# tambetm/simple_dqn

Measured on NVIDIA H100. Metric: DQN training steps/sec (batch 32, 84x84x4), higher is better.
Workload: dtype f16x3-split (fp32 accumulate)

## Files before the change

### simple_dqn_b200/csrc/net_umma.cu

```cuda
#include "net.cuh"
#include "net_umma.cuh"
#include "umma.cuh"
#include "umma2.cuh"
#include "umma_mn.cuh"
#include "conv1_tma.cuh"

namespace b200 {

__device__ __forceinline__ void ld8(const float* p, float v[8]) {
  const float4 a = *reinterpret_cast<const float4*>(p);
  const float4 b = *reinterpret_cast<const float4*>(p + 4);
  v[0] = a.x; v[1] = a.y; v[2] = a.z; v[3] = a.w; v[4] = b.x; v[5] = b.y; v[6] = b.z; v[7] = b.w;
}
__device__ __forceinline__ void st8(float* p, const float v[8]) {
  *reinterpret_cast<float4*>(p) = make_float4(v[0], v[1], v[2], v[3]);
  *reinterpret_cast<float4*>(p + 4) = make_float4(v[4], v[5], v[6], v[7]);
}
__device__ __forceinline__ void zero8(float v[8]) {
#pragma unroll
  for (int i = 0; i < 8; ++i) v[i] = 0.f;
}

struct UmmaState {
  __half* h16[3][2] = {};
  int64_t h_elems[3] = {};
  __half* dz16[4] = {};
  int64_t dz_elems[4] = {};
  uint8_t* img_fwd[2][4] = {};
  int64_t img_fwd_bytes[4] = {};
  uint8_t* im2col1 = nullptr;
  uint8_t* img_dgr[3] = {};
};
static inline UmmaState* ust(b200dqn_net* n) { return static_cast<UmmaState*>(n->umma_state); }

struct PlanePair {
  __half* hi;
  int64_t lo_off;
};

__device__ __forceinline__ void store_f32_and_planes(float* f32, const PlanePair& pl, int64_t i, const float v[8]) {
  if (f32) st8(f32 + i, v);
  umma2::split8_planes(v, pl.hi + i, pl.hi + pl.lo_off + i);
}

struct V2Conv1Fwd {
  static constexpr int kBN = 32;
  static constexpr bool kAExact = true, kARowMajorThreads = true, kBRowMajorThreads = false;
  static constexpr int kAMode = umma2::kReg, kBMode = umma2::kBulk;
  static constexpr bool kStagedEpilogue = true, kDumpA = true, kPrefetch = false;
  uint8_t* im2col;
  const uint8_t* src[2];
  const int32_t* idx[2];
  int shift[2];
  const uint8_t* wimg[2];
  float* out[2];
  PlanePair out16[2];
  int rows;
  __device__ int M(int) const { return rows * kP1 * kP1; }
  __device__ int N(int) const { return kC1; }
  __device__ void krange(int, int& kb, int& ke) const { kb = 0; ke = kK1 / 64; }
  __device__ const uint8_t* a_row_ptr(int z, int m) const {
    if (m >= rows * kP1 * kP1) return nullptr;
    const int n = m / (kP1 * kP1), pq = m % (kP1 * kP1), p = pq / kP1, q = pq % kP1;
    const int64_t f = static_cast<int64_t>((z ? idx[1] : idx[0])[n]) + (z ? shift[1] : shift[0]);
    return (z ? src[1] : src[0]) + f * kFrameBytes + (p * 4) * kFrameW + q * 4;
  }
  __device__ uint2 a_raw8(const uint8_t* row, int k0) const {
    if (!row) return make_uint2(0u, 0u);
    const int c = k0 >> 6, r = (k0 >> 3) & 7;
    const uint8_t* ptr = row + c * kFrameBytes + r * kFrameW;
    return make_uint2(*reinterpret_cast<const uint32_t*>(ptr), *reinterpret_cast<const uint32_t*>(ptr + 4));
  }
  __device__ static void cvt8(uint2 raw, float v[8]) {
#pragma unroll
    for (int j = 0; j < 4; ++j) {
      v[j] = float((raw.x >> (8 * j)) & 0xffu);
      v[4 + j] = float((raw.y >> (8 * j)) & 0xffu);
    }
  }
  __device__ const uint8_t* b_tile(int z, int, int kb) const { return (z ? wimg[1] : wimg[0]) + kb * (kC1 * 256); }
  __device__ uint8_t* a_dump(int z, int mtile, int kb) const {
    return (z == 0 && im2col) ? im2col + (int64_t(mtile) * (kK1 / 64) + kb) * (128 * 128) : nullptr;
  }
  __device__ void store8(int z, int m, int n0, const float v[8]) const {
    float o[8];
#pragma unroll
    for (int j = 0; j < 8; ++j) o[j] = fmaxf(v[j] * (1.0f / 255.0f), 0.f);
    store_f32_and_planes(z ? out[1] : out[0], z ? out16[1] : out16[0], int64_t(m) * kC1 + n0, o);
  }
};

template <int H, int C, int R, int ST, int KO>
struct V2ConvFwd {
  static constexpr int P = (H - R) / ST + 1, K = R * R * C;
  static_assert(K % 64 == 0 && C % 8 == 0, "k-blocks of 64, chunks of 8 channels");
  static constexpr int kBN = KO;
  static constexpr bool kAExact = false, kARowMajorThreads = true, kBRowMajorThreads = false;
  static constexpr int kAMode = umma2::kAsync, kBMode = umma2::kBulk;
  static constexpr bool kStagedEpilogue = true, kDumpA = false, kPrefetch = false;
  PlanePair in16[2];
  const uint8_t* wimg[2];
  float* out[2];
  PlanePair out16[2];
  int rows;
  __device__ int M(int) const { return rows * P * P; }
  __device__ int N(int) const { return KO; }
  __device__ void krange(int, int& kb, int& ke) const { kb = 0; ke = K / 64; }
  __device__ umma2::Planes a_planes(int z) const { return {z ? in16[1].hi : in16[0].hi, in16[0].lo_off}; }
  __device__ umma2::RowCtx a_row(int, int m) const {
    const int n = m / (P * P), pq = m % (P * P), p = pq / P, q = pq % P;
    return {(int64_t(n * H + p * ST) * H + q * ST) * C, 0, 0, m < rows * P * P};
  }
  __device__ bool a_chunk(int, const umma2::RowCtx& rc, int kk, int64_t& off) const {
    const int r = kk / (R * C), sc = kk % (R * C);
    off = rc.base + r * (H * C) + sc;
    return true;
  }
  __device__ const uint8_t* b_tile(int z, int, int kb) const { return (z ? wimg[1] : wimg[0]) + kb * (KO * 256); }
  __device__ void store8(int z, int m, int n0, const float v[8]) const {
    float o[8];
#pragma unroll
    for (int j = 0; j < 8; ++j) o[j] = fmaxf(v[j], 0.f);
    store_f32_and_planes(z ? out[1] : out[0], z ? out16[1] : out16[0], int64_t(m) * KO + n0, o);
  }
};

struct V2Fc1Fwd {
  static constexpr int kBN = 32;
  static constexpr bool kAExact = false, kARowMajorThreads = false, kBRowMajorThreads = true;
  static constexpr int kAMode = umma2::kBulk, kBMode = umma2::kAsync;
  static constexpr bool kStagedEpilogue = false, kDumpA = false, kPrefetch = false;
  static constexpr bool kAMnMajor = true;
  static constexpr uint32_t kAMnLoOffset = 128 * 128;
  PlanePair in16[2];
  const uint8_t* wimg[2];
  float* part;
  int rows, splits;
  __device__ int M(int) const { return kHidden; }
  __device__ int N(int) const { return rows; }
  __device__ void krange(int z, int& kb, int& ke) const {
    const int per = (kFlat / 64 + splits - 1) / splits;
    kb = (z % splits) * per;
    ke = min(kb + per, kFlat / 64);
  }
  __device__ const uint8_t* a_sub(int z, int mtile, int kb, int chunk) const {
    return ((z / splits) ? wimg[1] : wimg[0]) + (int64_t(kb >> 1) * (kHidden / 64) + 2 * mtile + chunk) * (128 * 256) +
           (kb & 1) * (64 * 128);
  }
  __device__ umma2::Planes b_planes(int z) const { return {(z / splits) ? in16[1].hi : in16[0].hi, in16[0].lo_off}; }
  __device__ umma2::RowCtx b_row(int, int n) const { return {int64_t(n) * kFlat, 0, 0, n < rows}; }
  __device__ bool b_chunk(int, const umma2::RowCtx& rc, int kk, int64_t& off) const {
    off = rc.base + kk;
    return true;
  }
  __device__ void store8(int z, int m, int n0, const float v[8]) const {
#pragma unroll
    for (int j = 0; j < 8; ++j)
      if (n0 + j < rows) part[(z * rows + n0 + j) * kHidden + m] = v[j];
  }
};

struct V2Fc1Dgrad {
  static constexpr int kBN = 32;
  static constexpr bool kAExact = false, kARowMajorThreads = true, kBRowMajorThreads = true;
  static constexpr int kAMode = umma2::kBulk, kBMode = umma2::kAsync;
  static constexpr bool kStagedEpilogue = false, kDumpA = false, kPrefetch = true;
  const uint8_t* wimg;
  PlanePair dz4;
  const float* h3;
  float* dz3;
  PlanePair dz3_16;
  int rows;
  __device__ int M(int) const { return kFlat; }
  __device__ int N(int) const { return rows; }
  __device__ void krange(int, int& kb, int& ke) const { kb = 0; ke = kHidden / 64; }
  __device__ const uint8_t* a_tile(int, int mtile, int kb) const {
    return wimg + (int64_t(mtile) * (kHidden / 64) + kb) * (128 * 256);
  }
  __device__ umma2::Planes b_planes(int) const { return {dz4.hi, dz4.lo_off}; }
  __device__ umma2::RowCtx b_row(int, int n) const { return {int64_t(n) * kHidden, 0, 0, n < rows}; }
  __device__ bool b_chunk(int, const umma2::RowCtx& rc, int kk, int64_t& off) const {
    off = rc.base + kk;
    return true;
  }
  __device__ void prefetch8(int, int m, int n0, float pf[8]) const {
#pragma unroll
    for (int j = 0; j < 8; ++j) pf[j] = (n0 + j < rows) ? h3[int64_t(n0 + j) * kFlat + m] : 0.f;
  }
  __device__ void store8p(int, int m, int n0, const float v[8], const float pf[8]) const {
#pragma unroll
    for (int j = 0; j < 8; ++j)
      if (n0 + j < rows) {
        const int64_t i = int64_t(n0 + j) * kFlat + m;
        const float o = pf[j] > 0.f ? v[j] : 0.f;
        if (dz3) dz3[i] = o;
        __half h, l;
        umma2::split1(o, h, l);
        dz3_16.hi[i] = h;
        dz3_16.hi[dz3_16.lo_off + i] = l;
      }
  }
};

template <int H, int C, int R, int ST, int KO, int STG = 0>
struct V2ConvDgrad {
  static constexpr int kStagesOverride = STG;
  static constexpr int P = (H - R) / ST + 1, RT = R / ST, HC = (H + ST - 1) / ST, K = RT * RT * KO;
  static_assert(K % 64 == 0 && KO % 8 == 0, "k-blocks of 64");
  static constexpr int kBN = C;
  static constexpr bool kAExact = false, kARowMajorThreads = true, kBRowMajorThreads = true;
  static constexpr int kAMode = umma2::kAsync, kBMode = umma2::kBulk;
  static constexpr bool kStagedEpilogue = true, kDumpA = false, kPrefetch = true;
  PlanePair dz;
  const uint8_t* wimg;
  const float* x;
  float* dx;
  PlanePair dx16;
  int rows;
  __device__ int M(int) const { return rows * HC * HC; }
  __device__ int N(int) const { return C; }
  __device__ void krange(int, int& kb, int& ke) const { kb = 0; ke = K / 64; }
  __device__ umma2::Planes a_planes(int) const { return {dz.hi, dz.lo_off}; }
  __device__ umma2::RowCtx a_row(int z, int m) const {
    const int n = m / (HC * HC), yx = m % (HC * HC), yy = yx / HC, xx = yx % HC;
    const bool ok = m < rows * HC * HC && yy * ST + z / ST < H && xx * ST + z % ST < H;
    return {(int64_t(n * P + yy) * P + xx) * KO, yy, xx, ok};
  }
  __device__ bool a_chunk(int, const umma2::RowCtx& rc, int kk, int64_t& off) const {
    const int rp = kk / (RT * KO), sp = (kk / KO) % RT, ko = kk % KO;
    const int p = rc.y - rp, q = rc.x - sp;
    off = rc.base - (rp * P + sp) * KO + ko;
    return p >= 0 && p < P && q >= 0 && q < P;
  }
  __device__ const uint8_t* b_tile(int z, int, int kb) const { return wimg + (int64_t(z) * (K / 64) + kb) * (C * 256); }
  __device__ void prefetch8(int z, int m, int c0, float pf[8]) const {
    const int n = m / (HC * HC), yx = m % (HC * HC), yy = yx / HC, xx = yx % HC;
    const int y = yy * ST + z / ST, xq = xx * ST + z % ST;
    if (y >= H || xq >= H) { zero8(pf); return; }
    ld8(x + (int64_t(n * H + y) * H + xq) * C + c0, pf);
  }
  __device__ void store8p(int z, int m, int c0, const float v[8], const float xv[8]) const {
    const int n = m / (HC * HC), yx = m % (HC * HC), yy = yx / HC, xx = yx % HC;
    const int y = yy * ST + z / ST, xq = xx * ST + z % ST;
    if (y >= H || xq >= H) return;
    const int64_t i = (int64_t(n * H + y) * H + xq) * C + c0;
    float o[8];
#pragma unroll
    for (int j = 0; j < 8; ++j) o[j] = xv[j] > 0.f ? v[j] : 0.f;
    if (dx) st8(dx + i, o);
    if (dx16.hi) umma2::split8_planes(o, dx16.hi + i, dx16.hi + dx16.lo_off + i);
  }
};

template <int H, int C, int R, int ST, int KO>
struct WConvWgrad {
  static constexpr int P = (H - R) / ST + 1, KW = R * R * C;
  static_assert((R * C) % 64 == 0 && KO == 64, "64-element runs must not straddle a filter row");
  static constexpr int kBN = 64, kStages = 4;
  static constexpr bool kAExact = false, kABulk = false;
  PlanePair x16;
  PlanePair dz16;
  float* part;
  int rows, kb_per_split;
  __device__ int M(int) const { return KW; }
  __device__ int N(int) const { return KO; }
  __device__ void krange(int z, int& kb, int& ke) const {
    const int total = (rows * P * P + 63) / 64;
    kb = min(z * kb_per_split, total);
    ke = min(kb + kb_per_split, total);
  }
  __device__ umma_mn::PixCtx pix(int, int kpix) const {
    const int n = kpix / (P * P), pq = kpix % (P * P);
    return {n, pq / P, pq % P, kpix < rows * P * P};
  }
  __device__ umma2::Planes a_planes(int) const { return {x16.hi, x16.lo_off}; }
  __device__ bool a_run(int, const umma_mn::PixCtx& px, int mchunk, int64_t& off) const {
    const int m = mchunk * 64, r = m / (R * C), sc = m % (R * C);
    off = (int64_t(px.n * H + px.p * ST + r) * H + px.q * ST) * C + sc;
    return m < KW;
  }
  __device__ umma2::Planes b_planes(int) const { return {dz16.hi, dz16.lo_off}; }
  __device__ int64_t b_off(int, const umma_mn::PixCtx& px) const { return (int64_t(px.n * P + px.p) * P + px.q) * KO; }
  __device__ void store8(int z, int m, int n0, const float v[8]) const { st8(part + (int64_t(z) * KW + m) * KO + n0, v); }
};

struct WConv1Wgrad {
  static constexpr int kBN = 32, kStages = 4;
  static constexpr bool kAExact = true, kABulk = true;
  const uint8_t* im2col;
  PlanePair dz16;
  float* part;
  int rows, kb_per_split;
  int tile_rows;
  __device__ int M(int) const { return kK1; }
  __device__ int N(int) const { return kC1; }
  __device__ int total_kb() const {
    return tile_rows == 128 ? (rows * kP1 * kP1 + 63) / 64 : rows * conv1tma::kTilesPerSample * 2;
  }
  __device__ void krange(int z, int& kb, int& ke) const {
    const int total = total_kb();
    kb = min(z * kb_per_split, total);
    ke = min(kb + kb_per_split, total);
  }
  __device__ umma_mn::PixCtx pix(int, int kpix) const {
    if (tile_rows == 128) return {kpix, 0, 0, kpix < rows * kP1 * kP1};
    const int tile = kpix >> 7, local = kpix & 127;
    return {tile * tile_rows + local, 0, 0, local < tile_rows && tile < rows * conv1tma::kTilesPerSample};
  }
  __device__ const uint8_t* a_sub(int, int c, int kb) const {
    return im2col + (int64_t(kb >> 1) * (kK1 / 64) + c) * (128 * 128) + (kb & 1) * (64 * 128);
  }
  __device__ umma2::Planes b_planes(int) const { return {dz16.hi, dz16.lo_off}; }
  __device__ int64_t b_off(int, const umma_mn::PixCtx& px) const { return int64_t(px.n) * kC1; }
  __device__ void store8(int z, int m, int n0, const float v[8]) const {
    float o[8];
#pragma unroll
    for (int j = 0; j < 8; ++j) o[j] = v[j] * (1.0f / 255.0f);
    st8(part + (int64_t(z) * kK1 + m) * kC1 + n0, o);
  }
};

struct WFc1Wgrad {
  static constexpr int kBN = 64, kStages = 2;
  static constexpr bool kAExact = false, kABulk = false;
  PlanePair h3_16;
  PlanePair dz4_16;
  float* dw4;
  int rows;
  __device__ int M(int) const { return kFlat; }
  __device__ int N(int) const { return kHidden; }
  __device__ void krange(int, int& kb, int& ke) const { kb = 0; ke = (rows + 63) / 64; }
  __device__ umma_mn::PixCtx pix(int, int b) const { return {b, 0, 0, b < rows}; }
  __device__ umma2::Planes a_planes(int) const { return {h3_16.hi, h3_16.lo_off}; }
  __device__ bool a_run(int, const umma_mn::PixCtx& px, int mchunk, int64_t& off) const {
    off = int64_t(px.n) * kFlat + mchunk * 64;
    return mchunk * 64 < kFlat;
  }
  __device__ umma2::Planes b_planes(int) const { return {dz4_16.hi, dz4_16.lo_off}; }
  __device__ int64_t b_off(int, const umma_mn::PixCtx& px) const { return int64_t(px.n) * kHidden; }
  __device__ void store8(int, int m, int n0, const float v[8]) const { st8(dw4 + int64_t(m) * kHidden + n0, v); }
};

struct WFc1WgradGather {
  static constexpr int kBN = 64, kStages = 2;
  static constexpr bool kAExact = false, kABulk = false;
  const __half* h3g;
  const __half* dzg;
  int64_t h3_parity, h3_lo, dz_parity, dz_lo;
  const uint32_t* epoch;
  float* dw4;
  int rows;
  __device__ int M(int) const { return kFlat; }
  __device__ int N(int) const { return kHidden; }
  __device__ void krange(int, int& kb, int& ke) const { kb = 0; ke = (rows + 63) / 64; }
  __device__ umma_mn::PixCtx pix(int, int b) const { return {b, 0, 0, b < rows}; }
  __device__ umma2::Planes a_planes(int) const { return {h3g + int64_t(epoch[0] & 1) * h3_parity, h3_lo}; }
  __device__ bool a_run(int, const umma_mn::PixCtx& px, int mchunk, int64_t& off) const {
    off = int64_t(px.n) * kFlat + mchunk * 64;
    return mchunk * 64 < kFlat;
  }
  __device__ umma2::Planes b_planes(int) const { return {dzg + int64_t(epoch[1] & 1) * dz_parity, dz_lo}; }
  __device__ int64_t b_off(int, const umma_mn::PixCtx& px) const { return int64_t(px.n) * kHidden; }
  __device__ void store8(int, int m, int n0, const float v[8]) const { st8(dw4 + int64_t(m) * kHidden + n0, v); }
};

template <int K, int N>
struct PackFwdConv {
  static constexpr bool kRowMajorThreads = false;
  const float* w;
  __host__ __device__ int tiles() const { return 1; }
  __host__ __device__ int rows() const { return N; }
  __host__ __device__ int kblocks() const { return K / 64; }
  __device__ void src8(int, int r, int k0, float v[8]) const {
#pragma unroll
    for (int j = 0; j < 8; ++j) v[j] = w[(k0 + j) * N + r];
  }
};
struct PackFc1Dgrad {
  static constexpr bool kRowMajorThreads = true;
  const float* w;
  __host__ __device__ int tiles() const { return (kFlat + 127) / 128; }
  __host__ __device__ int rows() const { return 128; }
  __host__ __device__ int kblocks() const { return kHidden / 64; }
  __device__ void src8(int tile, int r, int k0, float v[8]) const {
    const int m = tile * 128 + r;
    if (m >= kFlat) { zero8(v); return; }
    ld8(w + m * kHidden + k0, v);
  }
};
template <int H, int C, int R, int ST, int KO>
struct PackConvDgrad {
  static constexpr int RT = R / ST, K = RT * RT * KO;
  static constexpr bool kRowMajorThreads = true;
  const float* w;
  __host__ __device__ int tiles() const { return ST * ST; }
  __host__ __device__ int rows() const { return C; }
  __host__ __device__ int kblocks() const { return K / 64; }
  __device__ void src8(int z, int c, int k0, float v[8]) const {
    const int rp = k0 / (RT * KO), sp = (k0 / KO) % RT, ko = k0 % KO;
    const int r = rp * ST + z / ST, s = sp * ST + z % ST;
    ld8(w + ((r * R + s) * C + c) * KO + ko, v);
  }
};

template <int KR, int N, bool DGRAD, int C, int R, int ST, bool XCHG = false>
__global__ void __launch_bounds__(256)
k_opt_conv(const float* __restrict__ part, int splits, float* __restrict__ w, float* __restrict__ sst,
           uint8_t* __restrict__ img_fwd, uint8_t* __restrict__ img_dgr, const OptArgs opt, const XllArgs x,
           const KTrace kt) {
  constexpr int64_t kSize = int64_t(KR) * N;
  kt_begin(kt);
  pdl_wait();
  pdl_launch_dependents();
  const int tid = threadIdx.x, lane8 = tid & 7;
  uint32_t epoch = 0;
  if constexpr (XCHG) epoch = *reinterpret_cast<volatile uint32_t*>(x.epoch + x.chan) + 1;
  const int64_t e4 = blockIdx.x * 32 + (tid >> 3);
  const int64_t i = e4 * 4;
  const bool live = i < kSize;
  float4 g = make_float4(0.f, 0.f, 0.f, 0.f);
  if (live) {
    const float* p = part + i;
    float4 v[8];
    int cnt = 0;
#pragma unroll
    for (int u = 0; u < 8; ++u) {
      const int sp = lane8 + 8 * u;
      if (sp < splits) { v[u] = *reinterpret_cast<const float4*>(p + sp * kSize); cnt = u + 1; }
    }
    for (int u = 0; u < cnt; ++u) { g.x += v[u].x; g.y += v[u].y; g.z += v[u].z; g.w += v[u].w; }
  }
#pragma unroll
  for (int o = 1; o < 8; o <<= 1) {
    g.x += __shfl_xor_sync(0xffffffffu, g.x, o);
    g.y += __shfl_xor_sync(0xffffffffu, g.y, o);
    g.z += __shfl_xor_sync(0xffffffffu, g.z, o);
    g.w += __shfl_xor_sync(0xffffffffu, g.w, o);
  }
  if constexpr (XCHG) {
    float4 v = lane8 == x.rank ? g : make_float4(0.f, 0.f, 0.f, 0.f);
    if (live && lane8 < x.world && lane8 != x.rank) {
      const int64_t par = int64_t(epoch & 1) * x.world * x.lines_per_src, el = (x.ll4 + e4) * 2;
      uint4* dst = x.recv[lane8] + par + int64_t(x.rank) * x.lines_per_src + el;
      st_ll(dst, __float_as_uint(g.x), __float_as_uint(g.y), epoch);
      st_ll(dst + 1, __float_as_uint(g.z), __float_as_uint(g.w), epoch);
      const uint4* src = x.recv[x.rank] + par + int64_t(lane8) * x.lines_per_src + el;
      ll_wait(src, epoch, x.err, v.x, v.y);
      ll_wait(src + 1, epoch, x.err, v.z, v.w);
    }
    __syncwarp();
    const int base = (tid & 31) & ~7;
    g = make_float4(0.f, 0.f, 0.f, 0.f);
    for (int p = 0; p < x.world; ++p) {
      const float a = __shfl_sync(0xffffffffu, v.x, base + p), b = __shfl_sync(0xffffffffu, v.y, base + p);
      const float c = __shfl_sync(0xffffffffu, v.z, base + p), d = __shfl_sync(0xffffffffu, v.w, base + p);
      if (p == 0) g = make_float4(a, b, c, d);
      else { g.x += a; g.y += b; g.z += c; g.w += d; }
    }
  }
  if (live && lane8 == 0) {
    float wp[4];
    opt_update_vec<4>(opt, opt_step_scalar(opt), reinterpret_cast<const float*>(&g), wp, w + i, sst + i);
    __half hi[4], lo[4];
#pragma unroll
    for (int j = 0; j < 4; ++j) umma2::split1(wp[j], hi[j], lo[j]);
    const int k = int(i / N), n0 = int(i % N);
    {
      uint8_t* base = img_fwd + int64_t(k / 64) * (N * 256) + (k % 8) * 2;
      const int c8 = (k % 64) / 8;
#pragma unroll
      for (int j = 0; j < 4; ++j) {
        const uint32_t off = umma::sw128_off(n0 + j, c8);
        *reinterpret_cast<__half*>(base + off) = hi[j];
        *reinterpret_cast<__half*>(base + N * 128 + off) = lo[j];
      }
    }
    if constexpr (DGRAD) {
      constexpr int RT = R / ST, NKB = RT * RT * N / 64;
      const int r = k / (R * C), s = (k / C) % R, c = k % C;
      const int z = (r % ST) * ST + (s % ST);
      const int kd = ((r / ST) * RT + (s / ST)) * N + n0;
      uint8_t* base = img_dgr + (int64_t(z) * NKB + kd / 64) * (C * 256) + umma::sw128_off(c, (kd % 64) / 8) + (kd % 8) * 2;
      *reinterpret_cast<uint2*>(base) = *reinterpret_cast<const uint2*>(hi);
      *reinterpret_cast<uint2*>(base + C * 128) = *reinterpret_cast<const uint2*>(lo);
    }
  }
  if constexpr (XCHG) {
    __syncthreads();
    if (tid == 0) {
      __threadfence();
      if (atomicAdd(x.ticket + x.chan, 1u) == gridDim.x - 1) {
        x.ticket[x.chan] = 0;
        __threadfence();
        *reinterpret_cast<volatile uint32_t*>(x.epoch + x.chan) = epoch;
      }
    }
  }
  kt_end(kt);
}

__global__ void __launch_bounds__(256)
k_opt_fc1(const float* __restrict__ dw, float* __restrict__ w, float* __restrict__ sst, uint8_t* __restrict__ img_dgr,
          const OptArgs opt, const KTrace kt) {
  kt_begin(kt);
  pdl_wait();
  pdl_launch_dependents();
  constexpr int kNB = kHidden / 8;
  const float l_step = opt_step_scalar(opt);
  for (int id = blockIdx.x * blockDim.x + threadIdx.x; id < kFlat * kNB; id += gridDim.x * blockDim.x) {
    const int m = id / kNB, n0 = (id % kNB) * 8;
    const int64_t i = int64_t(m) * kHidden + n0;
    float g[8], wv[8];
    ld8(dw + i, g);
    opt_update_vec<8>(opt, l_step, g, wv, w + i, sst + i);
    uint4 hi, lo;
    umma::split8(wv, hi, lo);
    uint8_t* base = img_dgr + (int64_t(m / 128) * (kHidden / 64) + n0 / 64) * (128 * 256) +
                    umma::sw128_off(m % 128, (n0 % 64) / 8);
    *reinterpret_cast<uint4*>(base) = hi;
    *reinterpret_cast<uint4*>(base + 128 * 128) = lo;
  }
  kt_end(kt);
}

int umma_opt_fc1(b200dqn_net* n, int rows, cudaStream_t st, bool from_g) {
  UmmaState* u = ust(n);
  const LayerTable& lt = n->lt;
  const float* dw = from_g ? n->d_g + lt.off[3] : n->d_part + lt.part_off[3];
  const int ctas = 2 * n->sm_count;
  B2_CHECK_CUDA(launch_pdl(k_opt_fc1, dim3(ctas), dim3(256), 0, st, dw, n->d_w + lt.off[3],
                           n->d_s + lt.off[3], u->img_dgr[0], make_opt_args(n, rows), ktrace_slot("opt_fc1")));
  B2_PROF("opt_fc1", st);
  return B200DQN_OK;
}

int umma_opt_conv(b200dqn_net* n, int l, int rows, cudaStream_t st, const char* label, bool from_g) {
  UmmaState* u = ust(n);
  const LayerTable& lt = n->lt;
  const OptArgs opt = make_opt_args(n, rows);
  const float* part = from_g ? n->d_g + lt.off[l] : n->d_part + lt.part_off[l];
  const int nsplits = from_g ? 1 : lt.splits[l];
  float* w = n->d_w + lt.off[l];
  float* s = n->d_s + lt.off[l];
  B2_REQUIRE(nsplits <= 64, B200DQN_EINVAL, "k_opt_conv handles at most 64 split-K partials");
  const int64_t size = lt.off[l + 1] - lt.off[l];
  const dim3 grid(unsigned((size / 4 + 31) / 32)), block(256);
  cudaError_t e;
  const XllArgs none{};
  if (l == 0)
    e = launch_pdl(k_opt_conv<kK1, kC1, false, 4, 8, 4>, grid, block, 0, st, part, nsplits, w, s, u->img_fwd[0][0],
                   (uint8_t*)nullptr, opt, none, ktrace_slot(label));
  else if (l == 1)
    e = launch_pdl(k_opt_conv<kK2, kC2, true, kC1, 4, 2>, grid, block, 0, st, part, nsplits, w, s, u->img_fwd[0][1],
                   u->img_dgr[2], opt, none, ktrace_slot(label));
  else
    e = launch_pdl(k_opt_conv<kK3, kC3, true, kC2, 3, 1>, grid, block, 0, st, part, nsplits, w, s, u->img_fwd[0][2],
                   u->img_dgr[1], opt, none, ktrace_slot(label));
  B2_CHECK_CUDA(e);
  B2_PROF(label, st);
  return B200DQN_OK;
}

int umma_opt_conv_xll(b200dqn_net* n, int l, int rows, cudaStream_t st, const char* label) {
  UmmaState* u = ust(n);
  const LayerTable& lt = n->lt;
  const OptArgs opt = make_opt_args(n, rows);
  B2_REQUIRE(l >= 0 && l < 3 && lt.splits[l] <= 64 && n->world <= 8, B200DQN_EINVAL, "opt_conv_xll: bad layer / world");
  XllArgs x{};
  int rc = comm_xll_args(n, l, &x);
  if (rc) return rc;
  const float* part = n->d_part + lt.part_off[l];
  float* w = n->d_w + lt.off[l];
  float* s = n->d_s + lt.off[l];
  const int64_t size = lt.off[l + 1] - lt.off[l];
  const dim3 grid(unsigned((size / 4 + 31) / 32)), block(256);
  cudaError_t e;
  if (l == 0)
    e = launch_pdl(k_opt_conv<kK1, kC1, false, 4, 8, 4, true>, grid, block, 0, st, part, lt.splits[l], w, s,
                   u->img_fwd[0][0], (uint8_t*)nullptr, opt, x, ktrace_slot(label));
  else if (l == 1)
    e = launch_pdl(k_opt_conv<kK2, kC2, true, kC1, 4, 2, true>, grid, block, 0, st, part, lt.splits[l], w, s,
                   u->img_fwd[0][1], u->img_dgr[2], opt, x, ktrace_slot(label));
  else
    e = launch_pdl(k_opt_conv<kK3, kC3, true, kC2, 3, 1, true>, grid, block, 0, st, part, lt.splits[l], w, s,
                   u->img_fwd[0][2], u->img_dgr[1], opt, x, ktrace_slot(label));
  B2_CHECK_CUDA(e);
  B2_PROF(label, st);
  return B200DQN_OK;
}

static int64_t fwd_image_bytes(int layer) {
  switch (layer) {
    case 0: return int64_t(kK1 / 64) * kC1 * 256;
    case 1: return int64_t(kK2 / 64) * kC2 * 256;
    case 2: return int64_t(kK3 / 64) * kC3 * 256;
    default: return int64_t((kFlat + 127) / 128) * (kHidden / 64) * 128 * 256;
  }
}

int umma_pack_layers(b200dqn_net* n, int which, int l0, int l1, cudaStream_t st) {
  if (n->cfg.math_mode != B200DQN_MATH_TCGEN05) return B200DQN_OK;
  UmmaState* u = ust(n);
  const LayerTable& lt = n->lt;
  const float* w = which ? n->d_tw : n->d_w;
  int rc = 0;
  for (int l = l0; l <= l1 && !rc; ++l) {
    switch (l) {
      case 0: rc = umma2::launch_pack("pack_c1", PackFwdConv<kK1, kC1>{w + lt.off[0]}, u->img_fwd[which][0], st); break;
      case 1:
        rc = umma2::launch_pack("pack_c2f", PackFwdConv<kK2, kC2>{w + lt.off[1]}, u->img_fwd[which][1], st);
        if (!rc && !which)
          rc = umma2::launch_pack("pack_c2d", PackConvDgrad<kP1, kC1, 4, 2, kC2>{w + lt.off[1]}, u->img_dgr[2], st);
        break;
      case 2:
        rc = umma2::launch_pack("pack_c3f", PackFwdConv<kK3, kC3>{w + lt.off[2]}, u->img_fwd[which][2], st);
        if (!rc && !which)
          rc = umma2::launch_pack("pack_c3d", PackConvDgrad<kP2, kC2, 3, 1, kC3>{w + lt.off[2]}, u->img_dgr[1], st);
        break;
      case 3:
        rc = umma2::launch_pack("pack_fc1", PackFc1Dgrad{w + lt.off[3]}, u->img_fwd[which][3], st);
        break;
      default: break;
    }
  }
  return rc;
}

static inline int fc1_splits_for(int rows) {
  static const int forced = getenv("B200DQN_FC1_SPLITS") ? atoi(getenv("B200DQN_FC1_SPLITS")) : 0;
  if (forced >= 1 && forced <= kFc1Splits) return forced;
  return rows <= 256 ? 7 : 4;
}
constexpr int kUWgradKb = 4;

static const bool g_conv1_tma = getenv("B200DQN_CONV1") && strcmp(getenv("B200DQN_CONV1"), "tma") == 0;
static inline int conv1_pixels_padded(int rows) { return g_conv1_tma ? rows * conv1tma::kTilesPerSample * 128 : rows * kP1 * kP1; }

int umma_wgrad_kb(int layer, int rows) {
  const int kred = layer == 0 ? conv1_pixels_padded(rows) : layer == 1 ? rows * kP2 * kP2 : rows * kP3 * kP3;
  const int kbs = (kred + 63) / 64;
  int per = (kbs + 47) / 48;
  if (layer == 0 && per < 8) per = 8;
  return per > kUWgradKb ? per : kUWgradKb;
}
int umma_wgrad_splits(int layer, int rows) {
  const int kred = layer == 0 ? conv1_pixels_padded(rows) : layer == 1 ? rows * kP2 * kP2 : rows * kP3 * kP3;
  const int kbs = (kred + 63) / 64, per = umma_wgrad_kb(layer, rows);
  return (kbs + per - 1) / per;
}

int umma_net_init(b200dqn_net* n) {
  if (n->cfg.math_mode != B200DQN_MATH_TCGEN05) return B200DQN_OK;
  auto* u = new UmmaState();
  n->umma_state = u;
  const int nb = n->nb;
  u->h_elems[0] = int64_t(nb) * kP1 * kP1 * kC1;
  u->h_elems[1] = int64_t(nb) * kP2 * kP2 * kC2;
  u->h_elems[2] = int64_t(nb) * kFlat;
  u->dz_elems[0] = int64_t(nb) * kHidden;
  u->dz_elems[1] = int64_t(nb) * kFlat;
  u->dz_elems[2] = int64_t(nb) * kP2 * kP2 * kC2;
  u->dz_elems[3] = int64_t(nb) * kP1 * kP1 * kC1;
  for (int i = 0; i < 3; ++i) {
    for (int z = 0; z < 2; ++z) {
      B2_CHECK_CUDA(cudaMalloc(&u->h16[i][z], 2 * u->h_elems[i] * sizeof(__half)));
      B2_CHECK_CUDA(cudaMemset(u->h16[i][z], 0, 2 * u->h_elems[i] * sizeof(__half)));
    }
  }
  for (int i = 0; i < 4; ++i) {
    B2_CHECK_CUDA(cudaMalloc(&u->dz16[i], 2 * u->dz_elems[i] * sizeof(__half)));
    B2_CHECK_CUDA(cudaMemset(u->dz16[i], 0, 2 * u->dz_elems[i] * sizeof(__half)));
  }
  for (int l = 0; l < 4; ++l) {
    u->img_fwd_bytes[l] = fwd_image_bytes(l);
    for (int z = 0; z < 2; ++z) {
      if (z == 1 && n->d_tw == n->d_w) { u->img_fwd[1][l] = u->img_fwd[0][l]; continue; }
      B2_CHECK_CUDA(cudaMalloc(&u->img_fwd[z][l], u->img_fwd_bytes[l]));
      B2_CHECK_CUDA(cudaMemset(u->img_fwd[z][l], 0, u->img_fwd_bytes[l]));
    }
  }
  B2_CHECK_CUDA(cudaMalloc(&u->im2col1, int64_t((conv1_pixels_padded(nb) + 127) / 128) * (kK1 / 64) * 128 * 128));
  u->img_dgr[0] = u->img_fwd[0][3];
  const int64_t dgr_bytes[3] = {0, int64_t(kK3 / 64) * kC2 * 256, int64_t(4) * (256 / 64) * kC1 * 256};
  for (int i = 1; i < 3; ++i) {
    B2_CHECK_CUDA(cudaMalloc(&u->img_dgr[i], dgr_bytes[i]));
    B2_CHECK_CUDA(cudaMemset(u->img_dgr[i], 0, dgr_bytes[i]));
  }
  return B200DQN_OK;
}

void umma_net_destroy(b200dqn_net* n) {
  UmmaState* u = ust(n);
  if (!u) return;
  for (int i = 0; i < 3; ++i) {
    for (int z = 0; z < 2; ++z) cudaFree(u->h16[i][z]);
    if (i > 0) cudaFree(u->img_dgr[i]);
  }
  for (int i = 0; i < 4; ++i) cudaFree(u->dz16[i]);
  cudaFree(u->im2col1);
  for (int l = 0; l < 4; ++l) {
    if (u->img_fwd[1][l] != u->img_fwd[0][l]) cudaFree(u->img_fwd[1][l]);
    cudaFree(u->img_fwd[0][l]);
  }
  delete u;
  n->umma_state = nullptr;
}

int umma_weights_changed(b200dqn_net* n, cudaStream_t st) {
  if (n->cfg.math_mode != B200DQN_MATH_TCGEN05) return B200DQN_OK;
  int rc = umma_pack_layers(n, 0, 0, 3, st);
  if (!rc && n->d_tw != n->d_w) rc = umma_pack_layers(n, 1, 0, 3, st);
  return rc;
}

int umma_target_synced(b200dqn_net* n, cudaStream_t st) {
  if (n->cfg.math_mode != B200DQN_MATH_TCGEN05 || n->d_tw == n->d_w) return B200DQN_OK;
  UmmaState* u = ust(n);
  for (int l = 0; l < 4; ++l)
    B2_CHECK_CUDA(cudaMemcpyAsync(u->img_fwd[1][l], u->img_fwd[0][l], u->img_fwd_bytes[l], cudaMemcpyDeviceToDevice, st));
  return B200DQN_OK;
}

void umma_dz4_planes(b200dqn_net* n, __half** hi, int64_t* lo_off) {
  UmmaState* u = ust(n);
  *hi = u ? u->dz16[0] : nullptr;
  *lo_off = u ? u->dz_elems[0] : 0;
}

int umma_forward(b200dqn_net* n, const uint8_t* const src[2], const int32_t* const idx[2], const int shift[2],
                 const int64_t nframes[2], int nets, int rows, cudaStream_t st, bool release_early) {
  UmmaState* u = ust(n);
  int rc;
  auto planes = [&](int i, int z) { return PlanePair{u->h16[i][z], u->h_elems[i]}; };
  if (g_conv1_tma) {
    conv1tma::Params p{};
    const bool shared5 = nets == 2 && src[0] == src[1] && idx[0] == idx[1] && shift[1] == shift[0] + 1;
    for (int z = 0; z < 2; ++z) {
      p.idx[z] = idx[z]; p.shift[z] = shift[z];
      p.wimg[z] = u->img_fwd[z][0]; p.out16[z] = u->h16[0][z];
    }
    p.out[0] = n->d_h1[0];
    p.out[1] = nullptr;
    p.shared5 = shared5 ? 1 : 0; p.nets = nets; p.rows = rows; p.lo_off = u->h_elems[0];
    p.im2col = (nets == 2 && rows == n->nb) ? u->im2col1 : nullptr;
    CUtensorMap m0, m1;
    const int64_t nframes0 = nframes[0], nframes1 = nframes[1];
    if ((rc = conv1tma::make_frame_map(&m0, src[0], nframes0, shared5 ? kHist + 1 : kHist))) return rc;
    if ((rc = conv1tma::make_frame_map(&m1, src[nets == 2 ? 1 : 0], nets == 2 ? nframes1 : nframes0, kHist))) return rc;
    static bool configured = false;
    if (!configured) {
      B2_CHECK_CUDA(cudaFuncSetAttribute(conv1tma::k_conv1_tma, cudaFuncAttributeMaxDynamicSharedMemorySize,
                                         int(conv1tma::smem_bytes(2))));
      configured = true;
    }
    const uint32_t smem = conv1tma::smem_bytes((nets == 2 && !shared5) ? 2 : 1);
    B2_CHECK_CUDA(launch_pdl(conv1tma::k_conv1_tma, dim3(rows * conv1tma::kTilesPerSample), dim3(umma2::kThreads2),
                             smem, st, m0, m1, p, ktrace_slot("conv1_fwd")));
    B2_PROF("conv1_fwd", st);
  } else {
    V2Conv1Fwd p;
    for (int z = 0; z < 2; ++z) {
      p.src[z] = src[z]; p.idx[z] = idx[z]; p.shift[z] = shift[z];
      p.wimg[z] = u->img_fwd[z][0]; p.out[z] = n->d_h1[z]; p.out16[z] = planes(0, z);
    }
    p.rows = rows;
    p.im2col = (nets == 2 && rows == n->nb) ? u->im2col1 : nullptr;
    if ((rc = umma2::launch_umma2("conv1_fwd", p, rows * kP1 * kP1, kC1, nets, st, release_early))) return rc;
  }
  {
    using P = V2ConvFwd<kP1, kC1, 4, 2, kC2>;
    P p;
    for (int z = 0; z < 2; ++z) {
      p.in16[z] = planes(0, z); p.wimg[z] = u->img_fwd[z][1]; p.out16[z] = planes(1, z);
      p.out[z] = z ? nullptr : n->d_h2[z];
    }
    p.rows = rows;
    if ((rc = umma2::launch_umma2("conv2_fwd", p, rows * kP2 * kP2, kC2, nets, st, false))) return rc;
  }
  {
    using P = V2ConvFwd<kP2, kC2, 3, 1, kC3>;
    P p;
    for (int z = 0; z < 2; ++z) {
      p.in16[z] = planes(1, z); p.wimg[z] = u->img_fwd[z][2]; p.out16[z] = planes(2, z);
      p.out[z] = z ? nullptr : n->d_h3[z];
    }
    p.rows = rows;
    if ((rc = umma2::launch_umma2("conv3_fwd", p, rows * kP3 * kP3, kC3, nets, st, release_early))) return rc;
    if (nets == 2 && rows == n->nb && comm_gather_active(n, st) && (rc = umma_push_h3(n, st))) return rc;
  }
  {
    V2Fc1Fwd p;
    for (int z = 0; z < 2; ++z) { p.in16[z] = planes(2, z); p.wimg[z] = u->img_fwd[z][3]; }
    p.part = n->d_fc1part; p.rows = rows; p.splits = fc1_splits_for(rows);
    if ((rc = umma2::launch_umma2("fc1_fwd", p, kHidden, rows, nets * p.splits, st, false))) return rc;
  }
  return B200DQN_OK;
}

int umma_backward_op(b200dqn_net* n, int op, const uint8_t* src, const int32_t* idx, int shift, int rows,
                     cudaStream_t st, bool release_early) {
  const LayerTable& lt = n->lt;
  const float* w = n->d_w;
  switch (op) {
    case 0: {
      UmmaState* u = ust(n);
      WFc1Wgrad p{PlanePair{u->h16[2][0], u->h_elems[2]}, PlanePair{u->dz16[0], u->dz_elems[0]},
                  n->d_part + lt.part_off[3], rows};
      return umma_mn::launch_umma_mn("fc1_wgrad", p, kFlat, kHidden, 1, st, release_early);
    }
    case 1: {
      UmmaState* u = ust(n);
      V2Fc1Dgrad p{u->img_dgr[0], PlanePair{u->dz16[0], u->dz_elems[0]}, n->d_h3[0], n->keep_grads ? n->d_dz3 : nullptr,
                   PlanePair{u->dz16[1], u->dz_elems[1]}, rows};
      return umma2::launch_umma2("fc1_dgrad", p, kFlat, rows, 1, st, release_early);
    }
    case 2: {
      UmmaState* u = ust(n);
      using P = WConvWgrad<kP2, kC2, 3, 1, kC3>;
      P p{PlanePair{u->h16[1][0], u->h_elems[1]}, PlanePair{u->dz16[1], u->dz_elems[1]},
          n->d_part + lt.part_off[2], rows, umma_wgrad_kb(2, rows)};
      return umma_mn::launch_umma_mn("conv3_wgrad", p, P::KW, kC3, lt.splits[2], st, release_early);
    }
    case 3: {
      UmmaState* u = ust(n);
      using P = V2ConvDgrad<kP2, kC2, 3, 1, kC3>;
      P p{PlanePair{u->dz16[1], u->dz_elems[1]}, u->img_dgr[1], n->d_h2[0], n->keep_grads ? n->d_dz2 : nullptr,
          PlanePair{u->dz16[2], u->dz_elems[2]}, rows};
      return umma2::launch_umma2("conv3_dgrad", p, rows * P::HC * P::HC, kC2, 1, st, release_early);
    }
    case 4: {
      UmmaState* u = ust(n);
      using P = WConvWgrad<kP1, kC1, 4, 2, kC2>;
      P p{PlanePair{u->h16[0][0], u->h_elems[0]}, PlanePair{u->dz16[2], u->dz_elems[2]},
          n->d_part + lt.part_off[1], rows, umma_wgrad_kb(1, rows)};
      return umma_mn::launch_umma_mn("conv2_wgrad", p, P::KW, kC2, lt.splits[1], st, release_early);
    }
    case 5: {
      UmmaState* u = ust(n);
      using P = V2ConvDgrad<kP1, kC1, 4, 2, kC2>;
      using P2 = V2ConvDgrad<kP1, kC1, 4, 2, kC2, 2>;
      if (n->world == 1) {
        P2 p{PlanePair{u->dz16[2], u->dz_elems[2]}, u->img_dgr[2], n->d_h1[0], n->keep_grads ? n->d_dz1 : nullptr,
             PlanePair{u->dz16[3], u->dz_elems[3]}, rows};
        return umma2::launch_umma2("conv2_dgrad", p, rows * P::HC * P::HC, kC1, 4, st, release_early);
      }
      P p{PlanePair{u->dz16[2], u->dz_elems[2]}, u->img_dgr[2], n->d_h1[0], n->keep_grads ? n->d_dz1 : nullptr,
          PlanePair{u->dz16[3], u->dz_elems[3]}, rows};
      return umma2::launch_umma2("conv2_dgrad", p, rows * P::HC * P::HC, kC1, 4, st, release_early);
    }
    default: {
      UmmaState* u = ust(n);
      (void)src; (void)idx; (void)shift;
      WConv1Wgrad p{u->im2col1, PlanePair{u->dz16[3], u->dz_elems[3]}, n->d_part + lt.part_off[0], rows,
                    umma_wgrad_kb(0, rows), g_conv1_tma ? conv1tma::kTileRows : 128};
      return umma_mn::launch_umma_mn("conv1_wgrad", p, kK1, kC1, lt.splits[0], st, release_early);
    }
  }
}

int umma_fc1_splits(int rows) { return fc1_splits_for(rows); }
int umma_push_h3(b200dqn_net* n, cudaStream_t st) {
  UmmaState* u = ust(n);
  cudaStream_t sN = n->side[3];
  B2_CHECK_CUDA(cudaEventRecord(n->ev[13], st));
  B2_CHECK_CUDA(cudaStreamWaitEvent(sN, n->ev[13], 0));
  const int rc = comm_push_planes(n, 0, u->h16[2][0], u->h_elems[2], sN);
  if (rc) return rc;
  B2_CHECK_CUDA(cudaEventRecord(n->ev[14], sN));
  return B200DQN_OK;
}
int umma_push_dz4(b200dqn_net* n, cudaStream_t st) {
  UmmaState* u = ust(n);
  return comm_push_planes(n, 1, u->dz16[0], u->dz_elems[0], st);
}
int umma_gather_dz4_ll(b200dqn_net* n, cudaStream_t st) {
  UmmaState* u = ust(n);
  return comm_gather_dz4_ll(n, u->dz16[0], u->dz_elems[0], st, true);
}
int umma_fc1_wgrad_gathered(b200dqn_net* n, cudaStream_t st) {
  WFc1WgradGather p{reinterpret_cast<const __half*>(n->d_xbuf + n->x_h3_off),
                    reinterpret_cast<const __half*>(n->d_xbuf + n->x_dz_off),
                    n->x_h3_parity / 2, n->x_h3_lo, n->x_dz_parity / 2, n->x_dz_lo,
                    n->d_xpush_epoch, n->d_part + n->lt.part_off[3], n->nb * n->world};
  return umma_mn::launch_umma_mn("fc1_wgrad", p, kFlat, kHidden, 1, st, false);
}

}

extern "C" int b200dqn_debug_trace(unsigned long long* host_out, int n) {
  cudaDeviceSynchronize();
  return b200::umma2::read_trace(host_out, n);
}
```

Before: 10740.

## Fuse conv2 and conv3 forward into one per-sample kernel keeping h2 in shared memory

Adds a fused conv23 forward kernel that runs one block per sample and net. It computes conv2 with a pipelined wgmma ring, keeps the ReLU'd h2 hi/lo planes in shared memory, and streams the conv3 weights into the retired ring stages before running conv3 from shared memory. The aim is to remove one kernel launch and the global round trip of h2 for batches of up to 64 rows. In exchange each block uses a large amount of shared memory, the grid is only rows x nets blocks, and the h2 planes are written to global only for net 0.

```diff
diff --git a/simple_dqn_b200/csrc/net_umma.cu b/simple_dqn_b200/csrc/net_umma.cu
--- a/simple_dqn_b200/csrc/net_umma.cu
+++ b/simple_dqn_b200/csrc/net_umma.cu
@@ -124,6 +124,260 @@
     store_f32_and_planes(z ? out[1] : out[0], z ? out16[1] : out16[0], int64_t(m) * KO + n0, o);
   }
 };
+
+struct Conv23Fwd {
+  using C2 = V2ConvFwd<kP1, kC1, 4, 2, kC2>;
+  using C3 = V2ConvFwd<kP2, kC2, 3, 1, kC3>;
+  C2 c2;
+  C3 c3;
+};
+
+namespace conv23 {
+constexpr int kStages = 4;
+constexpr int kM2 = kP2 * kP2, kM3 = kP3 * kP3;
+constexpr int kKb2 = kK2 / 64, kKb3 = kK3 / 64;
+constexpr uint32_t kA2 = umma::kBM * 128;
+constexpr uint32_t kB2 = kC2 * 128;
+constexpr uint32_t kStage2 = 2 * kA2 + 2 * kB2;
+constexpr uint32_t kB3 = kC3 * 256;
+constexpr uint32_t kA3 = umma::kWgM * 128;
+constexpr uint32_t kStaging = 3 * kStage2;
+constexpr uint32_t kH2 = kStages * kStage2;
+constexpr uint32_t kPitch2 = kC2 * 4 + 16, kPitch3 = kC3 * 4 + 16;
+constexpr uint32_t kSmemBytes = kH2 + 2 * kM2 * 128 + 1024;
+static_assert(kKb3 * kB3 == 3 * kStage2, "stages 0-2 of the conv2 ring hold the nine conv3 weight images");
+static_assert(kStaging + umma::kBM * kPitch2 <= kH2 && kStaging + 3 * 2 * kA3 <= kH2, "stage 3: epilogue tile, A ring");
+static_assert(umma::kWgM * kPitch3 <= kStaging, "conv3 epilogue tile over the retired weight images");
+static_assert(kSmemBytes <= 227 * 1024, "H100: at most 227 KB of shared memory per block");
+}
+
+__global__ void __launch_bounds__(umma2::kThreads2, 1) k_conv23_fwd(const Conv23Fwd p, const int trace_in,
+                                                                    const KTrace kt) {
+  using namespace conv23;
+  using umma2::g_trace;
+  using umma2::kTraceSlots;
+  constexpr int S = kStages;
+  constexpr int kThreads = umma2::kThreads2;
+  extern __shared__ uint8_t smem_raw[];
+  __shared__ __align__(8) uint64_t s_full[S];
+  __shared__ __align__(8) uint64_t s_w3[kKb3];
+
+  const int tid = threadIdx.x, warp = tid >> 5, lane = tid & 31, wg = warp >> 2;
+  const int n = blockIdx.x, z = blockIdx.y;
+  const bool trace = trace_in && n == 0 && z == 0;
+  kt_begin(kt);
+  B2_TRACE(tid == 0, 0);
+  const uint32_t smem_base = (smem_u32(smem_raw) + 1023u) & ~1023u;
+  uint8_t* smem_gen = smem_raw + (smem_base - smem_u32(smem_raw));
+  uint8_t* h2 = smem_gen + kH2;
+  const uint8_t* wimg2 = z ? p.c2.wimg[1] : p.c2.wimg[0];
+  const uint8_t* wimg3 = z ? p.c3.wimg[1] : p.c3.wimg[0];
+
+  if (tid == 0) {
+#pragma unroll
+    for (int s = 0; s < S; ++s) mbar_init(&s_full[s], kThreads + 1);
+#pragma unroll
+    for (int kb = 0; kb < kKb3; ++kb) mbar_init(&s_w3[kb], 1);
+    mbar_fence_init();
+  }
+  __syncthreads();
+  B2_TRACE(tid == 0, 1);
+
+  constexpr int kACh = umma::kBM * 8 / kThreads;
+  umma2::RowCtx arow[kACh];
+  const umma2::Planes apl = p.c2.a_planes(z);
+#pragma unroll
+  for (int i = 0; i < kACh; ++i) {
+    const int m = (tid + i * kThreads) >> 3;
+    arow[i] = p.c2.a_row(z, n * kM2 + m);
+    arow[i].ok = m < kM2;
+  }
+  if (tid == 0) {
+#pragma unroll
+    for (int j = 0; j < S; ++j) {
+      mbar_arrive_expect_tx(&s_full[j], 2 * kB2);
+      tma_bulk_g2s(smem_gen + j * kStage2 + 2 * kA2, wimg2 + j * (2 * kB2), 2 * kB2, &s_full[j]);
+    }
+  }
+  pdl_wait();
+
+  auto stage2 = [&](int j) {
+    const int s = j % S, k0 = j * umma::kBK;
+    B2_TRACE(tid == 0, 8 + j * 4 + 2);
+    const uint32_t a_hi = smem_base + s * kStage2, a_lo = a_hi + kA2;
+    if (tid == 0 && j >= S) {
+      mbar_arrive_expect_tx(&s_full[s], 2 * kB2);
+      tma_bulk_g2s(smem_gen + s * kStage2 + 2 * kA2, wimg2 + j * (2 * kB2), 2 * kB2, &s_full[s]);
+    }
+#pragma unroll
+    for (int i = 0; i < kACh; ++i) {
+      const int id = tid + i * kThreads, r = id >> 3, c = id & 7;
+      int64_t eoff = 0;
+      const bool ok = arow[i].ok && p.c2.a_chunk(z, arow[i], k0 + c * 8, eoff);
+      const uint32_t bytes = ok ? 16u : 0u;
+      const __half* hi = apl.hi + (ok ? eoff : 0);
+      const uint32_t off = umma::sw128_off(r, c);
+      umma2::cp_async16(a_hi + off, hi, bytes);
+      umma2::cp_async16(a_lo + off, hi + apl.lo_off, bytes);
+    }
+    umma2::cp_async_arrive_noinc(&s_full[s]);
+    B2_TRACE(tid == 0, 8 + j * 4 + 3);
+  };
+  for (int j = 0; j < S; ++j) stage2(j);
+
+  float acc[kC2];
+  float acc2[kC2 / 2];
+#pragma unroll
+  for (int i = 0; i < kC2; ++i) acc[i] = 0.f;
+#pragma unroll
+  for (int i = 0; i < kC2 / 2; ++i) acc2[i] = 0.f;
+  for (int it = 0; it < kKb2; ++it) {
+    const int s = it % S;
+    mbar_wait(&s_full[s], (it / S) & 1);
+    fence_proxy_async_smem();
+    B2_TRACE(tid == 0, 8 + it * 4 + 0);
+    const uint32_t sa = smem_base + s * kStage2;
+    const uint64_t da_hi = umma::make_desc_sw128(sa + wg * umma::kWgM * 128);
+    const uint64_t da_lo = umma::make_desc_sw128(sa + kA2 + wg * umma::kWgM * 128);
+    const uint64_t db = umma::make_desc_sw128(sa + 2 * kA2);
+    umma::wgmma_fence();
+#pragma unroll
+    for (int k = 0; k < umma::kBK / 16; ++k) {
+      umma::wgmma_f16<2 * kC2>(acc, da_hi + 2 * k, db + 2 * k);
+      umma::wgmma_f16<kC2>(acc2, da_lo + 2 * k, db + 2 * k);
+    }
+    umma::wgmma_commit();
+    umma::wgmma_wait<1>();
+    B2_TRACE(tid == 0, 8 + it * 4 + 1);
+    if (it >= 1) {
+      umma2::named_bar_sync(1, kThreads);
+      const int freed = (it - 1) % S;
+      if (it - 1 + S < kKb2) {
+        stage2(it - 1 + S);
+      } else if (tid == 0) {
+#pragma unroll
+        for (int t = 0; t < 3; ++t) {
+          const int kb = 3 * freed + t;
+          mbar_arrive_expect_tx(&s_w3[kb], kB3);
+          tma_bulk_g2s(smem_gen + kb * kB3, wimg3 + kb * kB3, kB3, &s_w3[kb]);
+        }
+      }
+    }
+  }
+  B2_TRACE(tid == 0, 3);
+  pdl_launch_dependents();
+
+  umma::wgmma_wait<0>();
+  umma2::named_bar_sync(1, kThreads);
+  B2_TRACE(tid == 0, 4);
+  umma::stage_acc<kC2>(acc, acc2, smem_gen + kStaging, kPitch2, wg, warp, lane);
+  umma2::named_bar_sync(1, kThreads);
+  {
+    float* out = p.c2.out[0];
+    const PlanePair pl = p.c2.out16[0];
+#pragma unroll
+    for (int i = 0; i < umma::kBM * 8 / kThreads; ++i) {
+      const int id = tid + i * kThreads, r = id >> 3, cc = id & 7;
+      if (r < kM2) {
+        const uint8_t* src = smem_gen + kStaging + r * kPitch2 + cc * 32;
+        const float4 v0 = *reinterpret_cast<const float4*>(src), v1 = *reinterpret_cast<const float4*>(src + 16);
+        const float v[8] = {v0.x, v0.y, v0.z, v0.w, v1.x, v1.y, v1.z, v1.w};
+        float o[8];
+#pragma unroll
+        for (int j = 0; j < 8; ++j) o[j] = fmaxf(v[j], 0.f);
+        uint4 hi, lo;
+        umma::split8(o, hi, lo);
+        *reinterpret_cast<uint4*>(h2 + r * 128 + cc * 16) = hi;
+        *reinterpret_cast<uint4*>(h2 + kM2 * 128 + r * 128 + cc * 16) = lo;
+        if (z == 0) {
+          const int64_t e = int64_t(n * kM2 + r) * kC2 + cc * 8;
+          if (out) st8(out + e, o);
+          *reinterpret_cast<uint4*>(pl.hi + e) = hi;
+          *reinterpret_cast<uint4*>(pl.hi + pl.lo_off + e) = lo;
+        }
+      }
+    }
+  }
+  umma2::named_bar_sync(1, kThreads);
+  B2_TRACE(tid == 0, 2);
+
+  float acc3[kC3 / 2];
+  float acc3l[kC3 / 4];
+#pragma unroll
+  for (int i = 0; i < kC3 / 2; ++i) acc3[i] = 0.f;
+#pragma unroll
+  for (int i = 0; i < kC3 / 4; ++i) acc3l[i] = 0.f;
+  for (int it = 0; it < kKb3; ++it) {
+    const int r = it / 3, s = it % 3;
+    const uint32_t a_off = kStaging + (it % 3) * (2 * kA3);
+    B2_TRACE(tid == 0, 8 + (kKb2 + it) * 4 + 2);
+#pragma unroll
+    for (int i = 0; i < umma::kWgM * 8 / kThreads; ++i) {
+      const int id = tid + i * kThreads, m = id >> 3, c = id & 7;
+      uint4 hi = make_uint4(0u, 0u, 0u, 0u), lo = hi;
+      if (m < kM3) {
+        const int src = (m / kP3 + r) * kP2 + m % kP3 + s;
+        hi = *reinterpret_cast<const uint4*>(h2 + src * 128 + c * 16);
+        lo = *reinterpret_cast<const uint4*>(h2 + kM2 * 128 + src * 128 + c * 16);
+      }
+      *reinterpret_cast<uint4*>(smem_gen + a_off + umma::sw128_off(m, c)) = hi;
+      *reinterpret_cast<uint4*>(smem_gen + a_off + kA3 + umma::sw128_off(m, c)) = lo;
+    }
+    fence_proxy_async_smem();
+    umma2::named_bar_sync(1, kThreads);
+    mbar_wait(&s_w3[it], 0);
+    B2_TRACE(tid == 0, 8 + (kKb2 + it) * 4 + 0);
+    const uint64_t da_hi = umma::make_desc_sw128(smem_base + a_off);
+    const uint64_t da_lo = umma::make_desc_sw128(smem_base + a_off + kA3);
+    const uint32_t b = smem_base + it * kB3 + wg * 32 * 128;
+    const uint64_t db_hi = umma::make_desc_sw128(b), db_lo = umma::make_desc_sw128(b + kC3 * 128);
+    umma::wgmma_fence();
+#pragma unroll
+    for (int k = 0; k < umma::kBK / 16; ++k) {
+      umma::wgmma_f16<32>(acc3, da_hi + 2 * k, db_hi + 2 * k);
+      umma::wgmma_f16<32>(acc3 + kC3 / 4, da_hi + 2 * k, db_lo + 2 * k);
+      umma::wgmma_f16<32>(acc3l, da_lo + 2 * k, db_hi + 2 * k);
+    }
+    umma::wgmma_commit();
+    umma::wgmma_wait<1>();
+    B2_TRACE(tid == 0, 8 + (kKb2 + it) * 4 + 1);
+  }
+
+  umma::wgmma_wait<0>();
+  umma2::named_bar_sync(1, kThreads);
+  B2_TRACE(tid == 0, 7);
+  umma::stage_acc<32>(acc3, acc3l, smem_gen + wg * 32 * 4, kPitch3, 0, warp, lane);
+  umma2::named_bar_sync(1, kThreads);
+#pragma unroll
+  for (int i = 0; i < umma::kWgM * 8 / kThreads; ++i) {
+    const int id = tid + i * kThreads, m = id >> 3, cc = id & 7;
+    if (m < kM3) {
+      const uint8_t* src = smem_gen + m * kPitch3 + cc * 32;
+      const float4 v0 = *reinterpret_cast<const float4*>(src), v1 = *reinterpret_cast<const float4*>(src + 16);
+      const float v[8] = {v0.x, v0.y, v0.z, v0.w, v1.x, v1.y, v1.z, v1.w};
+      p.c3.store8(z, n * kM3 + m, cc * 8, v);
+    }
+  }
+  B2_TRACE(tid == 0, 5);
+  kt_end(kt);
+  B2_TRACE(tid == 0, 6);
+}
+
+constexpr int kConv23MaxRows = 64;
+
+static int launch_conv23(const Conv23Fwd& p, int rows, int nets, cudaStream_t st) {
+  static bool configured = false;
+  if (!configured) {
+    B2_CHECK_CUDA(cudaFuncSetAttribute(k_conv23_fwd, cudaFuncAttributeMaxDynamicSharedMemorySize, conv23::kSmemBytes));
+    configured = true;
+  }
+  static const char* trace_label = getenv("B200DQN_TRACE_LABEL");
+  const int trace = (trace_label && strcmp(trace_label, "conv23_fwd") == 0) ? 1 : 0;
+  B2_CHECK_CUDA(launch_pdl(k_conv23_fwd, dim3(rows, nets), dim3(umma2::kThreads2), conv23::kSmemBytes, st, p, trace,
+                           ktrace_slot("conv23_fwd")));
+  B2_PROF("conv23_fwd", st);
+  return B200DQN_OK;
+}
 
 struct V2Fc1Fwd {
   static constexpr int kBN = 32;
@@ -767,27 +1021,39 @@
     p.im2col = (nets == 2 && rows == n->nb) ? u->im2col1 : nullptr;
     if ((rc = umma2::launch_umma2("conv1_fwd", p, rows * kP1 * kP1, kC1, nets, st, release_early))) return rc;
   }
-  {
-    using P = V2ConvFwd<kP1, kC1, 4, 2, kC2>;
-    P p;
+  if (rows <= kConv23MaxRows) {
+    Conv23Fwd p{};
     for (int z = 0; z < 2; ++z) {
-      p.in16[z] = planes(0, z); p.wimg[z] = u->img_fwd[z][1]; p.out16[z] = planes(1, z);
-      p.out[z] = z ? nullptr : n->d_h2[z];
-    }
-    p.rows = rows;
-    if ((rc = umma2::launch_umma2("conv2_fwd", p, rows * kP2 * kP2, kC2, nets, st, false))) return rc;
-  }
-  {
-    using P = V2ConvFwd<kP2, kC2, 3, 1, kC3>;
-    P p;
-    for (int z = 0; z < 2; ++z) {
-      p.in16[z] = planes(1, z); p.wimg[z] = u->img_fwd[z][2]; p.out16[z] = planes(2, z);
-      p.out[z] = z ? nullptr : n->d_h3[z];
-    }
-    p.rows = rows;
-    if ((rc = umma2::launch_umma2("conv3_fwd", p, rows * kP3 * kP3, kC3, nets, st, release_early))) return rc;
-    if (nets == 2 && rows == n->nb && comm_gather_active(n, st) && (rc = umma_push_h3(n, st))) return rc;
-  }
+      p.c2.in16[z] = planes(0, z); p.c2.wimg[z] = u->img_fwd[z][1];
+      p.c3.wimg[z] = u->img_fwd[z][2]; p.c3.out16[z] = planes(2, z);
+      p.c3.out[z] = z ? nullptr : n->d_h3[z];
+    }
+    p.c2.out[0] = n->d_h2[0]; p.c2.out16[0] = planes(1, 0);
+    p.c2.rows = p.c3.rows = rows;
+    if ((rc = launch_conv23(p, rows, nets, st))) return rc;
+  } else {
+    {
+      using P = V2ConvFwd<kP1, kC1, 4, 2, kC2>;
+      P p;
+      for (int z = 0; z < 2; ++z) {
+        p.in16[z] = planes(0, z); p.wimg[z] = u->img_fwd[z][1]; p.out16[z] = planes(1, z);
+        p.out[z] = z ? nullptr : n->d_h2[z];
+      }
+      p.rows = rows;
+      if ((rc = umma2::launch_umma2("conv2_fwd", p, rows * kP2 * kP2, kC2, nets, st, false))) return rc;
+    }
+    {
+      using P = V2ConvFwd<kP2, kC2, 3, 1, kC3>;
+      P p;
+      for (int z = 0; z < 2; ++z) {
+        p.in16[z] = planes(1, z); p.wimg[z] = u->img_fwd[z][2]; p.out16[z] = planes(2, z);
+        p.out[z] = z ? nullptr : n->d_h3[z];
+      }
+      p.rows = rows;
+      if ((rc = umma2::launch_umma2("conv3_fwd", p, rows * kP3 * kP3, kC3, nets, st, release_early))) return rc;
+    }
+  }
+  if (nets == 2 && rows == n->nb && comm_gather_active(n, st) && (rc = umma_push_h3(n, st))) return rc;
   {
     V2Fc1Fwd p;
     for (int z = 0; z < 2; ++z) { p.in16[z] = planes(2, z); p.wimg[z] = u->img_fwd[z][3]; }
```

Result: faster. 11080, median of 6 (+3.2%).
